# pchero/asterisk-tiresias

Hardware: AMD Instinct MI355X
Metric: fingerprints/sec + match latency p50, 8 kHz mono, 1/2/4/8 MI355X (higher is better)
Workload: dtype f32

## Files before the change

asterisk-tiresias_amd/csrc/tfp_kernels.hip:

```cpp
#include <hip/hip_runtime.h>
#include <hipcub/hipcub.hpp>
#include <type_traits>

#include "tfp_kernels.hpp"
#include "tfp_log.hpp"
#include "tfp_math.hpp"
#include "tfp_split.hpp"
#include "tfp_synth.hpp"

namespace tfp {


typedef float cf __attribute__((ext_vector_type(2)));

__device__ __forceinline__ cf swap(cf a) { return __builtin_shufflevector(a, a, 1, 0); }
__device__ __forceinline__ cf addsub(cf c, cf p) { return __builtin_elementwise_fma(p, cf{1.f, -1.f}, c); }
__device__ __forceinline__ cf subadd(cf c, cf p) { return __builtin_elementwise_fma(p, cf{-1.f, 1.f}, c); }

__device__ __forceinline__ cf cmul(cf a, cf w) {
  const cf p = a * cf{w.x, w.x};
  const cf q = swap(a) * cf{w.y, w.y};
  return subadd(p, q);
}

// ... 486 lines not shown
        micro[2 * g + cf] = micro_of_db(q);
        if (db) db[2 * g + cf] = q;
      }
    }
    wave_sync();
    if (__builtin_expect(dense_rows != 0, 0)) {
      const float lempty = aubio_log10_fast(0.f, S.logf);
      for (int i = lane; i < kWaveFrames * kFilters; i += 64) {
        const int r = i / kFilters, j = i % kFilters;
        if (((dense_rows >> r) & 1u) && T->mel_len[j] == 0) M.logs[r * kLogStride + j] = lempty;
      }
      dense_rows = 0;
      wave_sync();
    }
    c = cn;
    f0 = fn0;
  }
}

__device__ __forceinline__ void dft4_rot_a2(cf a0, cf a1, cf A2, cf a3, cf& X0, cf& X1, cf& X2, cf& X3) {
  const cf t0 = addsub(a0, swap(A2)), t1 = subadd(a0, swap(A2)), t2 = a1 + a3, t3 = a1 - a3;
  X0 = t0 + t2;
  X2 = t0 - t2;
  X1 = addsub(t1, swap(t3));
  X3 = subadd(t1, swap(t3));
}
__device__ __forceinline__ cf cmul_w2(cf a, float c) {
  const cf p = a * cf{c, c};
  return addsub(p, swap(p));
}
__device__ __forceinline__ cf cmul_w6(cf a, float d) {
  const cf p = a * cf{d, d};
  return subadd(p, swap(p));
}
__device__ __forceinline__ void dft16q(const cf (&w16)[10], const cf (&in)[16], cf (&out)[16]) {
  cf A[4][4];
#pragma unroll
  for (int n2 = 0; n2 < 4; n2++) dft4(in[n2], in[4 + n2], in[8 + n2], in[12 + n2], A[n2][0], A[n2][1], A[n2][2], A[n2][3]);
#pragma unroll
  for (int n2 = 1; n2 < 4; n2++)
#pragma unroll
    for (int k1 = 1; k1 < 4; k1++) {
      const int e = n2 * k1;
      if (e == 2) A[n2][k1] = cmul_w2(A[n2][k1], w16[2].x);
      else if (e == 6) A[n2][k1] = cmul_w6(A[n2][k1], w16[6].x);
      else if (e != 4) A[n2][k1] = cmul(A[n2][k1], w16[e]);
    }
#pragma unroll
  for (int k1 = 0; k1 < 4; k1++) {
    if (k1 == 2) dft4_rot_a2(A[0][k1], A[1][k1], A[2][k1], A[3][k1], out[k1], out[k1 + 4], out[k1 + 8], out[k1 + 12]);
    else dft4(A[0][k1], A[1][k1], A[2][k1], A[3][k1], out[k1], out[k1 + 4], out[k1 + 8], out[k1 + 12]);
  }
}

template <int LEN>
__device__ __forceinline__ float mel_sum_w(const float* __restrict__ N, const float4 (&wv)[LEN / 4], int st) {
  float4 nv[LEN / 4];
#pragma unroll
  for (int i = 0; i < LEN / 4; i++) nv[i] = *reinterpret_cast<const float4*>(N + st + 4 * i);
  float acc = 0.f;
#pragma unroll
  for (int i = 0; i < LEN / 4; i++) {
    const cf p01 = cf{nv[i].x, nv[i].y} * cf{wv[i].x, wv[i].y};
    const cf p23 = cf{nv[i].z, nv[i].w} * cf{wv[i].z, wv[i].w};
    acc = i == 0 ? p01.x : acc + p01.x;
    acc = acc + p01.y; acc = acc + p23.x; acc = acc + p23.y;
  }
  return acc;
}
template <int LEN>
__device__ __forceinline__ void load_w(const float* __restrict__ w, float4 (&wv)[LEN / 4]) {
#pragma unroll
  for (int i = 0; i < LEN / 4; i++) wv[i] = *reinterpret_cast<const float4*>(w + 64 * i);
}

#ifdef TFP_STAMPS
#define TFP_STAMP(i) const uint64_t ts##i = __builtin_amdgcn_s_memtime()
#define TFP_ACC(i, a, b) st[i] += ts##b - ts##a
#else
#define TFP_STAMP(i)
#define TFP_ACC(i, a, b)
#endif

template <int kPasses>
__global__ __launch_bounds__(64 * fp8_block_waves<kPasses>(), TFP_FP_WAVES) void fingerprint8k_kernel(
    const DspTables* __restrict__ T, const int16_t* __restrict__ pcm, const int64_t* __restrict__ sbeg,
    const int64_t* __restrict__ send, const int64_t* __restrict__ foff, const int32_t* __restrict__ toff,
    const int32_t* __restrict__ tclip, int32_t ntiles, int32_t* __restrict__ micro, double* __restrict__ db,
    float rare_thr, LogFix fx, int64_t single_ns) {
  constexpr int LA = 36, LB = 16, LC = 8;
  constexpr bool kSplitTail = kPasses >= 2;
#ifdef TFP_STAMPS
  const uint64_t t_entry = __builtin_amdgcn_s_memtime();
#endif
  const uint32_t rare_m1 = __builtin_bit_cast(uint32_t, rare_thr) - 1u;
  constexpr bool kPairFb = kPasses >= 2;
  constexpr int kBW = fp8_block_waves<kPasses>();
  using WaveT = WaveLds8;
  __shared__ __attribute__((aligned(16))) LdsTables S;
  __shared__ __attribute__((aligned(16))) WaveT WL[kBW];
  const int tid = threadIdx.x;
  const int wave = __builtin_amdgcn_readfirstlane(tid >> 6);
  const int lane = tid & 63, grp = lane >> 4, L = lane & 15;
  struct Tile {
    int c;
    int64_t f0, s0, ns;
    __amdgpu_buffer_rsrc_t rs;
    bool odd;
  };
  auto clip_rsrc = [&](int64_t s0, int64_t ns) {
    const uintptr_t a = reinterpret_cast<uintptr_t>(pcm + s0);
    const int16_t* base = reinterpret_cast<const int16_t*>(a & ~(uintptr_t)3);
    const int64_t bytes = (2 * ns + (int64_t)(a & 3) + 3) & ~(int64_t)3;
    return __builtin_amdgcn_make_buffer_rsrc(const_cast<int16_t*>(base), (short)0, (int)bytes, 0x00020000);
  };
  auto tile_of = [&](int b) {
    Tile t;
    if (single_ns >= 0) {
      t.c = 0;
      t.f0 = (int64_t)b * (4 * kPasses);
      t.s0 = 0;
      t.ns = single_ns;
    } else {
      t.c = __builtin_amdgcn_readfirstlane(tclip[b]);
      t.f0 = (int64_t)(b - toff[t.c]) * (4 * kPasses);
      t.s0 = sbeg[t.c];
      t.ns = send[t.c] - t.s0;
    }
    if constexpr (kPairFb) {
      t.rs = clip_rsrc(t.s0, t.ns);
      t.odd = (reinterpret_cast<uintptr_t>(pcm + t.s0) & 3) != 0;
    }
    return t;
  };
  auto fetch = [&](const Tile& t, int sub, bool valid, int4 (&pf)[kChunkRounds]) {
    const int16_t* clip = pcm + t.s0;
    const int64_t sb = (t.f0 + 4 * sub - 1) * kHop;
    const bool interior = valid && ((reinterpret_cast<uintptr_t>(clip) & 15) == 0) && sb >= 0 && sb + kPassSamples <= t.ns;
    if (interior) {
      const int4* src = reinterpret_cast<const int4*>(clip + sb);
#pragma unroll
      for (int r = 0; r < kChunkRounds; r++) {
        const int chunk = lane + 64 * r;
        pf[r] = (64 * r + 63 < kPassChunks || chunk < kPassChunks) ? src[chunk] : make_int4(0, 0, 0, 0);
      }
    } else if constexpr (kPasses == 1) {
      const bool aligned = (reinterpret_cast<uintptr_t>(clip) & 15) == 0;
#pragma unroll
      for (int r = 0; r < kChunkRounds; r++) {
        const int chunk = lane + 64 * r;
        const int64_t s0 = sb + 8 * chunk;
        int4 v = make_int4(0, 0, 0, 0);
        if (valid && chunk < kPassChunks && s0 + 8 > 0 && s0 < t.ns) {
          if (aligned && s0 >= 0 && s0 + 8 <= t.ns) v = *reinterpret_cast<const int4*>(clip + s0);
          else v = fetch_chunk_inline(clip, t.ns, s0);
        }
        pf[r] = v;
      }
    } else {
#pragma unroll
      for (int r = 0; r < kChunkRounds; r++) {
        const int chunk = lane + 64 * r;
        pf[r] = (valid && chunk < kPassChunks) ? fetch_chunk_checked(clip, t.ns, sb + 8 * chunk) : make_int4(0, 0, 0, 0);
      }
    }
  };

  auto fetchd = [&](const Tile& t, int sub, uint32_t (&pw)[16]) {
    if (t.odd) return;
    const __amdgpu_buffer_rsrc_t rs = t.rs;
    const int32_t fs = (int32_t)((t.f0 + 4 * sub - 1 + grp) * kHop) + 2 * L;
#pragma unroll
    for (int n1 = 0; n1 < 16; n1++) {
      const int32_t j = n1 < 8 ? 256 + 32 * n1 : 32 * (n1 - 8);
      pw[n1] = __builtin_amdgcn_raw_buffer_load_b32(rs, 2 * (fs + j), 0, 0);
    }
  };

  int4 pf[kChunkRounds];
  uint32_t pw[16];
  int b = blockIdx.x * kBW + wave;
  Tile cur = tile_of(b < ntiles ? b : 0);
  cf* winr = reinterpret_cast<cf*>(S.window);
  cf* twr = S.tw512;
  constexpr int kStage = 256;
  const int ts = tid < kStage ? tid : kStage - 1;
  const bool stager = tid < kStage;
  constexpr int kMsW = kPairFb ? kFbSteps * kFbPatterns : 16 * (LA + LB + LC);
  const float* const wsrc = kPairFb ? &T->fb_w[0][0][0] : T->ms_w;
  const int wL = (ts >> 1) & 15, wn1 = 2 * (ts >> 5) + (ts & 1);
  const int wj = (32 * wn1 + 2 * wL + 256) & 511;
  const float win0 = T->window_s[wj], win1 = T->window_s[wj + 1];
  const int tk2 = ts >> 5, tkk = (wL == 0 && tk2 == 0) ? 128 : wL + 16 * tk2;
  const float* tws = (ts & 1) ? T->tw512_im : T->tw512_re;
  const float twk = tws[tkk], twk2 = tws[256 - tkk];
  const int li = ts < 240 ? ts : 239, lk1 = 1 + li / 16, lL = li % 16;
  const float ltre = T->lane_tw_re[lk1][lL], ltim = T->lane_tw_im[lk1][lL];
  const int i10 = ts < 10 ? ts : 9;
  const float w16re = T->tw256_re[16 * i10], w16im = T->tw256_im[16 * i10];
  const int i80 = ts < kCoefs * kFilters ? ts : kCoefs * kFilters - 1;
  const float dctv = (&T->dct[0][0])[i80];
  const int i48 = ts < 48 ? ts : 47;
  const int msf = (&T->ms_filter[0][0])[i48], mss = (&T->ms_start[0][0])[i48];
  const int i3 = ts < 3 ? ts : 2;
  const int msl = T->ms_len[i3], mso = T->ms_woff[i3];
  const LogfEntry lge = logf_table()[ts & 15];
  float mw[(kMsW + kStage - 1) / kStage];
#pragma unroll
  for (int r = 0; r < (kMsW + kStage - 1) / kStage; r++) {
    int idx = ts + kStage * r;
    idx = idx < kMsW ? idx : kMsW - 1;
    if constexpr (kPairFb) {
      const int q = idx & 3, pat = (idx >> 2) & 15, s4 = idx >> 6;
      idx = ((2 * s4 + (q >> 1)) * kFbPatterns + pat) * 2 + (q & 1);
    }
    mw[r] = wsrc[idx];
  }
  const int mlen = T->mel_len[lane < kFilters ? lane : kFilters - 1];
  if constexpr (kPairFb) fetchd(cur, 0, pw);
  else fetch(cur, 0, b < ntiles, pf);
  if (stager) {
    winr[tid] = cf{win0, win1};
    twr[tid] = cf{twk, twk2};
  if (tid < 240) S.lane_tw[lk1 - 1][lL] = cf{ltre, ltim};
  if (tid < 10) S.w16[tid] = cf{w16re, w16im};
  if (tid < kCoefs * kFilters) (&S.dct[0][0])[tid] = dctv;
  if (tid < 48) {
    (&S.ms_filter[0][0])[tid] = msf;
    (&S.ms_start[0][0])[tid] = mss;
  }
  if (tid < 3) { S.ms_len[tid] = msl; S.ms_woff[tid] = mso; }
  if (tid < 16) S.logf[tid] = lge;
  if (kPairFb && tid < kLogf2Entries) S.logf2[tid] = logf2_entry(tid, logf_table());
  if (tid == 0) { S.c_defer = T->ms_c_defer; S.c_real[0] = T->ms_c_real[0]; S.c_real[1] = T->ms_c_real[1]; }
#pragma unroll
    for (int r = 0; r < (kMsW + kStage - 1) / kStage; r++) {
      const int idx = tid + kStage * r;
      if (idx < kMsW) S.ms_w[idx] = 0.5f * mw[r];
    }
  }
  const unsigned long long empty_filters = __ballot(lane < kFilters && mlen == 0);
  __syncthreads();
#ifdef TFP_STAMPS
  const uint64_t t_staged = __builtin_amdgcn_s_memtime();
#endif

  WaveT& M = WL[wave];
  cf* W = M.scratch[grp];
  float* N = reinterpret_cast<float*>(W) + 48 * (grp & 1);
  const int nwaves = gridDim.x * kBW;
  const int maxbin = T->ms_maxbin;
  const int fA = S.ms_filter[0][L], fB = S.ms_filter[1][L], fC = S.ms_filter[2][L];
  const bool c_real = fC >= 0 && (fC == S.c_real[0] || fC == S.c_real[1]);
  cf w16r[10];
#pragma unroll
  for (int e = 0; e < 10; e++)
    w16r[e] = cf{T->tw256_re[16 * e], T->tw256_im[16 * e]};
  cf ltw[15];
#pragma unroll
  for (int k1 = 1; k1 < 16; k1++) ltw[k1 - 1] = S.lane_tw[k1 - 1][L];
  const float lempty = aubio_log10_fast(0.f, S.logf);
  if constexpr (!kPairFb) {
    for (int i = lane; i < 4 * kPasses * kFilters; i += 64) {
      const int j = i % kFilters;
      if ((empty_filters >> j) & 1) M.logs[(i / kFilters) * kLogStride + j] = lempty;
    }
  }
  const float* fbb[kFbSegs];
  float* fbc[kFbSegs];
  float fbk[kFbSegs];
  cf dctl, dct9;
  const float* const fbrow = (grp < 2 ? M.xeven : reinterpret_cast<const float*>(M.scratch)) + (grp & 1) * kFbRow;
  float* const fblog = M.logs + 4 * grp * kFbNf;
  if constexpr (kPairFb) {
    const int lf = lane < kFbNf ? lane : lane - kFbNf, l9 = kFbNf - 4 + (lane & 3);
    dctl = cf{S.dct[0][lf], S.dct[1][lf]};
    dct9 = cf{S.dct[0][l9], S.dct[1][l9]};
#pragma unroll
    for (int k = 0; k < kFbSegs; k++) {
      fbb[k] = fbrow + 2 * (T->fb_bin[L][k] - kFbSegStart[k]);
      fbc[k] = fblog + T->fb_filter[L][k];
      fbk[k] = T->fb_new[L][k] ? 0.f : 1.f;
    }
  }

#ifdef TFP_STAMPS
  uint64_t st[7] = {0, 0, 0, 0, 0, 0, 0};
  uint64_t tprev = __builtin_amdgcn_s_memtime();
  const uint64_t tstart = tprev;
  int npass = 0;
#endif
  for (; b < ntiles; b += nwaves) {
    const int64_t nf = (cur.ns + kHop - 1) / kHop;
    const int bn = b + nwaves;
    const Tile nxt = bn < ntiles ? tile_of(bn) : cur;

    for (int sub = 0; sub < kPasses; sub++) {
      const int row = sub * 4 + grp;
      int oz = 0;
      asm volatile("" : "+v"(oz));
      wave_sync();
      TFP_STAMP(0);
      cf wreg[16];
#pragma unroll
      for (int i = 0; i < 8; i++) {
        const float4 w4 = *reinterpret_cast<const float4*>(winr + (i * 16 + L) * 2 + oz);
        wreg[2 * i] = cf{w4.x, w4.y};
        wreg[2 * i + 1] = cf{w4.z, w4.w};
      }
      if constexpr (!kPairFb) {
#pragma unroll
        for (int r = 0; r < kChunkRounds; r++) {
          const int chunk = lane + 64 * r;
          if (chunk < kPassChunks) *reinterpret_cast<int4*>(M.pcm + (chunk >> 5) * kHopStride + (chunk & 31) * 8) = pf[r];
        }
        if (sub < kPasses - 1) fetch(cur, sub + 1, true, pf);
        else fetch(nxt, 0, bn < ntiles, pf);
      }
      wave_sync();
      TFP_STAMP(1);
      const int16_t* hop0 = M.pcm + grp * kHopStride;
      cf z[16], Y[16];
      if constexpr (kPairFb) {
        const int64_t pb = (cur.f0 + 4 * sub - 1) * kHop;
        const int32_t fs = (int32_t)(pb + grp * kHop) + 2 * L;
        if (cur.odd) {
          const __amdgpu_buffer_rsrc_t rs = cur.rs;
#pragma unroll
          for (int n1 = 0; n1 < 16; n1++) {
            const int32_t j = n1 < 8 ? 256 + 32 * n1 : 32 * (n1 - 8);
            const uint32_t lo = __builtin_amdgcn_raw_buffer_load_b32(rs, 2 * (fs + j), 0, 0);
            const uint32_t hi = __builtin_amdgcn_raw_buffer_load_b32(rs, 2 * (fs + j) + 4, 0, 0);
            pw[n1] = (lo >> 16) | (hi << 16);
          }
        }
        if (pb < 0 || pb + kPassSamples > cur.ns) {
#pragma unroll
          for (int n1 = 0; n1 < 16; n1++) {
            const int32_t s0 = fs + (n1 < 8 ? 256 + 32 * n1 : 32 * (n1 - 8));
            const uint32_t lo = (s0 >= 0 && s0 < cur.ns) ? 0xffffu : 0u;
            const uint32_t hi = (s0 + 1 >= 0 && s0 + 1 < cur.ns) ? 0xffff0000u : 0u;
            pw[n1] &= lo | hi;
          }
        }
      }
#pragma unroll
      for (int n1 = 0; n1 < 16; n1++) {
        int32_t v;
        if constexpr (kPairFb) {
          v = (int32_t)pw[n1];
        } else {
          const int j = (32 * n1 + 2 * L + 256) & 511;
          const int hsel = n1 < 8 ? 1 : 0;
          v = *reinterpret_cast<const int32_t*>(hop0 + hsel * kHopStride + (j & 255));
        }
        z[n1] = cf{(float)(int16_t)(v & 0xffff), (float)(int16_t)(v >> 16)} * wreg[n1];
      }
      if constexpr (kPairFb) {
        if (sub < kPasses - 1) fetchd(cur, sub + 1, pw);
        else fetchd(nxt, 0, pw);
      }
      dft16q(w16r, z, Y);
#pragma unroll
      for (int k1 = 1; k1 < 16; k1++) Y[k1] = cmul(Y[k1], ltw[k1 - 1]);
      wave_sync();
      TFP_STAMP(2);
// ... 115 lines not shown
              if (st == 0) acc = p0;
              else if (st == kFbSegStart[k]) acc = __builtin_elementwise_fma(acc, cf{jk[k], jk[k]}, p0);
              else acc = acc + p0;
              acc = acc + p1;
            }
            seg[k] = acc;
          };
          using I0 = std::integral_constant<int, 0>;
          using I1 = std::integral_constant<int, 1>;
          using I2 = std::integral_constant<int, 2>;
          using I3 = std::integral_constant<int, 3>;
          static_assert(kFbSegs == 4, "four segments");
          load_seg(I0{});
          load_seg(I1{});
          asm volatile("" ::: "memory");
          sum_seg(I0{});
          load_seg(I2{});
          asm volatile("" ::: "memory");
          sum_seg(I1{});
          load_seg(I3{});
          asm volatile("" ::: "memory");
          sum_seg(I2{});
          sum_seg(I3{});
#pragma unroll
          for (int k = 0; k < kFbSegs; k++) {
            jc[k][doff] = seg[k].x;
            jc[k][doff + 2 * kFbNf] = seg[k].y;
          }
        };
        if (sub == 1) pair_fb(std::integral_constant<int, 0>{});
        else pair_fb(std::integral_constant<int, 1>{});
      }
#ifdef TFP_STAMPS
      const uint64_t ts5 = __builtin_amdgcn_s_memtime();
      st[0] += ts0 - tprev;
      TFP_ACC(1, 0, 1);
      TFP_ACC(2, 1, 2);
      TFP_ACC(3, 2, 3);
      TFP_ACC(4, 3, 4);
      TFP_ACC(5, 4, 5);
      tprev = ts5;
      npass++;
#endif
    }
    wave_sync();
    if constexpr (kPairFb) {
      constexpr int kFull = 8;
      static_assert(kWaveFrames * kFbNf == kFull * 2 * kFbNf && 2 * kFbNf - 64 == 4, "log rounds");
      cf* const prod = reinterpret_cast<cf*>(M.scratch);
      LogArg g[kFull];
      LogfEntry en[kFull];
#pragma unroll
      for (int r = 0; r < kFull; r++) g[r] = log_reduce(M.logs[2 * kFbNf * r + lane]);
#pragma unroll
      for (int r = 0; r < kFull; r++) en[r] = S.logf2[g[r].idx];
#pragma unroll
      for (int r = 0; r < kFull; r++) {
        const float l = log_finish(g[r], en[r]);
        prod[2 * kFbNf * r + lane] = cf{l, l} * dctl;
      }
      if (lane < kWaveFrames * 2) {
        const int i = 2 * kFbNf * (lane >> 2) + 64 + (lane & 3);
        const float l = aubio_log10_frexp(M.logs[i], S.logf2);
        prod[i] = cf{l, l} * dct9;
      }
    } else if (lane < 2 * 4 * kPasses) {
      const int f = S.c_real[lane & 1];
      if (f >= 0) {
        float* p = M.logs + (lane >> 1) * kLogStride + f;
        *p = aubio_log10_fast(*p, S.logf);
      }
    }
    wave_sync();
    if (lane < 2 * 4 * kPasses) {
      const int row = lane >> 1, cfi = lane & 1;
      const int64_t f = cur.f0 + row;
      if (f < nf) {
        float acc = 0.f;
        if constexpr (kPairFb) {
          const float* prow = reinterpret_cast<const float*>(M.scratch) + 2 * (2 * (row & 7) + (row >> 3)) * kFbNf + cfi;
#pragma unroll
          for (int i = 0; i < kFbNf; i++) acc = acc + prow[2 * i];
#pragma unroll
          for (int i = kFbNf; i < kFilters; i++) acc = acc + lempty * S.dct[cfi][i];
        } else {
          const float* lrow = M.logs + row * kLogStride;
#pragma unroll 8
          for (int i = 0; i < kFilters; i++) acc = acc + lrow[i] * S.dct[cfi][i];
        }
        const int64_t g = (single_ns >= 0 ? 0 : foff[cur.c]) + f;
        if constexpr (kSplitTail) {
          micro[2 * g + cfi] = __builtin_bit_cast(int32_t, acc);
        } else {
          const double q = db ? db_of_coef(acc, fx) : db_of_coef(acc);
          micro[2 * g + cfi] = micro_of_db(q);
          if (db) db[2 * g + cfi] = q;
        }
      }
    }
    wave_sync();
    cur = nxt;
  }
#ifdef TFP_STAMPS
  const uint64_t t_end = __builtin_amdgcn_s_memtime();
  if (lane == 0 && (blockIdx.x & 63) == 0)
    printf("stamps<%d> block %d wave %d passes %d | entry->staged %lu staged->loop %lu loop %lu after-last-pass %lu | "
           "lead %lu stage %lu fft1 %lu fft2 %lu split %lu mel %lu\n",
           kPasses, (int)blockIdx.x, wave, npass, (unsigned long)(t_staged - t_entry), (unsigned long)(tstart - t_staged),
           (unsigned long)(tprev - tstart), (unsigned long)(t_end - tprev), (unsigned long)st[0], (unsigned long)st[1],
           (unsigned long)st[2], (unsigned long)st[3], (unsigned long)st[4], (unsigned long)st[5]);
#endif
}

__global__ void finish_db_kernel(int32_t* __restrict__ micro, double* __restrict__ db, int64_t nvals, LogFix fx) {
  for (int64_t i = (int64_t)blockIdx.x * blockDim.x + threadIdx.x; i < nvals; i += (int64_t)gridDim.x * blockDim.x) {
    const float c = __builtin_bit_cast(float, micro[i]);
    const double q = db ? db_of_coef(c, fx) : db_of_coef(c);
    micro[i] = micro_of_db(q);
    if (db) db[i] = q;
  }
}

bool DspTables_fixed8k(const DspTables& t) {
  return t.ms_len[0] == 36 && t.ms_len[1] == 16 && t.ms_len[2] == 8 && t.ms_total == 16 * (36 + 16 + 8) &&
         t.ms_total <= kMsLds && t.ms_c_defer == 1 && t.ms_maxbin <= 2 * kFrameStride8 - 48 &&
         t.ms_filter[0][15] >= 0 && t.ms_filter[1][15] >= 0 && t.fb_ok == 1 && t.fb_nfilters == kFbNf &&
         t.tw256_im[32] == -t.tw256_re[32] && t.tw256_im[96] == t.tw256_re[96];
}

static int resident_blocks(const void* k, int waves = kBlockWaves) {
  int per = 0;
  (void)hipOccupancyMaxActiveBlocksPerMultiprocessor(&per, k, 64 * waves, 0);
  hipFuncAttributes a;
  if (hipFuncGetAttributes(&a, k) == hipSuccess) {
    const int vg = ((a.numRegs > 0 ? a.numRegs : 1) + 7) / 8 * 8;
    int by_vgpr = 512 / vg;
    if (by_vgpr > 8) by_vgpr = 8;
    by_vgpr = by_vgpr * 4 / waves;
    const int by_lds = a.sharedSizeBytes ? (int)((160 * 1024) / a.sharedSizeBytes) : 8;
    const int own = by_vgpr < by_lds ? by_vgpr : by_lds;
    if (per <= 0 || own < per) per = own;
  }
  return per > 0 ? per : 1;
}

hipError_t fp_launch_config(int device, FpLaunchCfg* cfg) {
  int cus = 0;
  hipError_t e = hipDeviceGetAttribute(&cus, hipDeviceAttributeMultiprocessorCount, device);
  if (e != hipSuccess) return e;
  auto cap = [&](const void* k, int waves = kBlockWaves) { return cus * resident_blocks(k, waves); };
  cfg->grid_cap_8k = cap(reinterpret_cast<const void*>(fingerprint8k_kernel<kTile8k / 4>), kBW8);
  cfg->grid_cap_8k_small = cap(reinterpret_cast<const void*>(fingerprint8k_kernel<1>));
  cfg->grid_cap_generic = cap(reinterpret_cast<const void*>(fingerprint_kernel<int16_t>));
  cfg->grid_cap_f32 = cap(reinterpret_cast<const void*>(fingerprint_kernel<float>));
  if (knob("TFP_DEBUG_OCC")) {
    int per = 0;
    (void)hipOccupancyMaxActiveBlocksPerMultiprocessor(&per, reinterpret_cast<const void*>(fingerprint8k_kernel<kTile8k / 4>),
                                                       64 * kBW8, 0);
    fprintf(stderr, "[tfp] fingerprint8k_kernel<%d>: %d blocks/CU (occupancy query %d), grid cap %d\n", kTile8k / 4,
            cfg->grid_cap_8k / cus, per, cfg->grid_cap_8k);
    hipFuncAttributes fa;
    if (hipFuncGetAttributes(&fa, reinterpret_cast<const void*>(fingerprint8k_kernel<kTile8k / 4>)) == hipSuccess)
      fprintf(stderr, "[tfp]   %d threads/block (max %d), %d VGPRs, %zu B LDS, %zu B scratch\n", 64 * kBW8,
              fa.maxThreadsPerBlock, fa.numRegs, fa.sharedSizeBytes, fa.localSizeBytes);
    int smem = 0, smem_optin = 0;
    (void)hipDeviceGetAttribute(&smem, hipDeviceAttributeMaxSharedMemoryPerBlock, device);
    (void)hipDeviceGetAttribute(&smem_optin, hipDeviceAttributeSharedMemPerBlockOptin, device);
    fprintf(stderr, "[tfp]   device: %d B LDS per block (opt-in %d)\n", smem, smem_optin);
  }
  if (const char* b = knob("TFP_FP_BLOCKS_PER_CU")) {
    const int n = atoi(b);
    if (n > 0 && cus * n < cfg->grid_cap_8k) cfg->grid_cap_8k = cus * n;
  }
  const char* g = knob("TFP_GENERIC");
  cfg->force_generic = g && atoi(g);
  const char* rt = knob("TFP_RARE_THR_LOG2");
  int rl = rt ? atoi(rt) : -98;
  rl = rl < -98 ? -98 : (rl > 100 ? 100 : rl);
  cfg->rare_thr = ldexpf(1.f, rl);
  return hipSuccess;
}

hipError_t launch_fingerprint(const FpLaunchCfg& cfg, const DspTables* d_tables, bool fixed8k, int32_t tile_frames,
                              const int16_t* d_pcm, const int64_t* d_sbeg, const int64_t* d_send, const int64_t* d_foff,
                              const int32_t* d_toff, const int32_t* d_tclip, int32_t ntiles, int64_t nframes,
                              int32_t* d_micro, double* d_db, hipStream_t s, const LogFix& fx, FpLaunchStats* stats,
                              int64_t single_ns) {
  const bool v8 = fixed8k && (tile_frames == 4 || !cfg.force_generic);
  if (v8 ? !(tile_frames == 4 || tile_frames == kTile8k) : tile_frames != kFramesPerBlock) return hipErrorInvalidValue;
  if (ntiles <= 0) return hipSuccess;
  const int cap = v8 ? (tile_frames == 4 ? cfg.grid_cap_8k_small : cfg.grid_cap_8k) : cfg.grid_cap_generic;
  if (cap <= 0) return hipErrorInvalidValue;
  const int bw = (v8 && tile_frames != 4) ? kBW8 : kBlockWaves;
  const int want = (ntiles + bw - 1) / bw;
  const int grid = want < cap ? want : cap;
  if (v8) {
    if (tile_frames == 4) {
      hipLaunchKernelGGL(fingerprint8k_kernel<1>, dim3(grid), dim3(kBlockThreads), 0, s, d_tables, d_pcm, d_sbeg, d_send,
                         d_foff, d_toff, d_tclip, ntiles, d_micro, d_db, cfg.rare_thr, fx, single_ns);
      if (stats) stats->small8k++;
    } else {
      hipLaunchKernelGGL(fingerprint8k_kernel<kTile8k / 4>, dim3(grid), dim3(64 * kBW8), 0, s, d_tables, d_pcm, d_sbeg,
                         d_send, d_foff, d_toff, d_tclip, ntiles, d_micro, d_db, cfg.rare_thr, fx, single_ns);
      if (stats) stats->throughput8k++;
      if (const hipError_t le = hipGetLastError(); le != hipSuccess) return le;
      const int64_t nv = 2 * nframes;
      int64_t g = (nv + 255) / 256;
      if (g > 8192) g = 8192;
      if (nv > 0) hipLaunchKernelGGL(finish_db_kernel, dim3((unsigned)g), dim3(256), 0, s, d_micro, d_db, nv, fx);
    }
    return hipGetLastError();
  }
  hipLaunchKernelGGL(fingerprint_kernel<int16_t>, dim3(grid), dim3(kBlockThreads), 0, s, d_tables, d_pcm, d_sbeg, d_send,
                     d_foff, d_toff, d_tclip, ntiles, d_micro, d_db, fx);
  if (stats) stats->generic_i16++;
  return hipGetLastError();
}

hipError_t launch_fingerprint_f32(const FpLaunchCfg& cfg, const DspTables* d_tables, const float* d_x,
                                  const int64_t* d_sbeg, const int64_t* d_send, const int64_t* d_foff,
                                  const int32_t* d_toff, const int32_t* d_tclip, int32_t ntiles, int32_t* d_micro,
                                  double* d_db, hipStream_t s, const LogFix& fx, FpLaunchStats* stats) {
  if (ntiles <= 0) return hipSuccess;
  if (cfg.grid_cap_f32 <= 0) return hipErrorInvalidValue;
  const int want = (ntiles + kBlockWaves - 1) / kBlockWaves;
  const int grid = want < cfg.grid_cap_f32 ? want : cfg.grid_cap_f32;
  hipLaunchKernelGGL(fingerprint_kernel<float>, dim3(grid), dim3(kBlockThreads), 0, s, d_tables, d_x, d_sbeg, d_send,
                     d_foff, d_toff, d_tclip, ntiles, d_micro, d_db, fx);
  if (stats) stats->generic_f32++;
  return hipGetLastError();
}

__global__ void synth_kernel(const SynthSpecDev* __restrict__ specs, int64_t spc, int16_t* __restrict__ out) {
  const int c = blockIdx.y;
  const SynthSpecDev sp = specs[c];
  const SynthClip p = synth_clip(sp.seed, sp.clip);
  for (int64_t s = (int64_t)blockIdx.x * blockDim.x + threadIdx.x; s < spc; s += (int64_t)gridDim.x * blockDim.x)
    out[(int64_t)c * spc + s] = synth_sample(p, sp.offset + s);
}

hipError_t launch_synth(const SynthSpecDev* d_specs, int32_t nclips, int64_t spc, int16_t* d_out, hipStream_t s) {
  if (nclips <= 0 || spc <= 0) return hipSuccess;
  int64_t bx = (spc + 255) / 256;
  if (bx > 256) bx = 256;
  hipLaunchKernelGGL(synth_kernel, dim3((unsigned)bx, nclips), dim3(256), 0, s, d_specs, spc, d_out);
  return hipGetLastError();
}

__global__ void index_keys_kernel(const int32_t* __restrict__ m1, const int32_t* __restrict__ clip,
                                  const int32_t* __restrict__ rank, int64_t n, int32_t* keys, int32_t* vals) {
  for (int64_t i = (int64_t)blockIdx.x * blockDim.x + threadIdx.x; i < n; i += (int64_t)gridDim.x * blockDim.x) {
    const int32_t v = m1[i];
    const bool live = rank[clip[i]] >= 0 && v != kNullMicro;
    keys[i] = live ? v : INT32_MAX;
    vals[i] = (int32_t)i;
  }
}

hipError_t launch_index_keys(const int32_t* st_m1, const int32_t* st_clip, const int32_t* rank_of_clip, int64_t n,
                             int32_t* keys, int32_t* vals, hipStream_t s) {
  if (n <= 0) return hipSuccess;
  hipLaunchKernelGGL(index_keys_kernel, dim3(2048), dim3(256), 0, s, st_m1, st_clip, rank_of_clip, n, keys, vals);
  return hipGetLastError();
}

__global__ void index_gather_kernel(const int32_t* __restrict__ sv, const int32_t* __restrict__ m2,
                                    const int32_t* __restrict__ clip, const int32_t* __restrict__ rank, int64_t n,
                                    int32_t* m2s, int32_t* cols) {
  for (int64_t i = (int64_t)blockIdx.x * blockDim.x + threadIdx.x; i < n; i += (int64_t)gridDim.x * blockDim.x) {
    const int32_t j = sv[i];
    m2s[i] = m2[j];
    cols[i] = rank[clip[j]];
  }
}

hipError_t launch_index_gather(const int32_t* sorted_vals, const int32_t* st_m2, const int32_t* st_clip,
                               const int32_t* rank_of_clip, int64_t n, int32_t* m2s, int32_t* cols, hipStream_t s) {
  if (n <= 0) return hipSuccess;
  hipLaunchKernelGGL(index_gather_kernel, dim3(2048), dim3(256), 0, s, sorted_vals, st_m2, st_clip, rank_of_clip, n,
                     m2s, cols);
  return hipGetLastError();
}

__device__ __forceinline__ int64_t lower_bound_i32(const int32_t* a, int64_t n, int64_t v) {
  int64_t lo = 0, hi = n;
  while (lo < hi) {
// ... 811 lines not shown
```

asterisk-tiresias_amd/csrc/tfp_kernels.hpp:

```cpp
#pragma once
#include <hip/hip_runtime.h>
#include <stdint.h>
#include <stdlib.h>
#include <string.h>

#include "tfp_math.hpp"
#include "tfp_tables.hpp"

namespace tfp {

inline const char* knob(const char* name) {
  const char* on = getenv("TFP_TEST_KNOBS");
  return on && *on && strcmp(on, "0") != 0 ? getenv(name) : nullptr;
}
inline const char* op_env(const char* name) {
  const char* v = getenv(name);
  return v && *v ? v : nullptr;
}

constexpr int kFramesPerBlock = 16;
constexpr int kTile8k = 16;
constexpr int64_t kDirectMaxSamples = (int64_t(1) << 30) - (int64_t(1) << 16);
constexpr int32_t kKeyOffset = 512;
constexpr int32_t kKeyRange = 1024;

struct FrameBox {
  int64_t L1, U1, L2, U2;
  int32_t k;
  int32_t flags;
};

struct SearchConsts {
  int32_t coefs;
  int32_t has_low, has_high;
  int32_t pad;
  double tole, thr_low, thr_high;
};

#ifdef __HIPCC__
__device__ __forceinline__ bool frame_key(const double* __restrict__ q, int64_t i, const SearchConsts& sc, int32_t& k) {
  const double q1 = q[2 * i];
  const double v1 = __builtin_isfinite(q1) ? q1 : 0.0;
  k = (v1 > -2147483649.0 && v1 < 2147483648.0) ? (int32_t)v1 : INT32_MIN;
  const double freq = (double)k;
  if (sc.has_low && freq < sc.thr_low) return false;
  if (sc.has_high && freq > sc.thr_high) return false;
  return __builtin_isfinite(freq - sc.tole) && __builtin_isfinite(freq + sc.tole);
}

__device__ __forceinline__ FrameBox frame_box(double q1, double q2, const SearchConsts& sc) {
  const double v1 = __builtin_isfinite(q1) ? q1 : 0.0;
  const int32_t ki = (v1 > -2147483649.0 && v1 < 2147483648.0) ? (int32_t)v1 : INT32_MIN;
  const double freq = (double)ki;
  FrameBox bx;
  bx.k = ki;
  bx.flags = 1;
  bx.L2 = bx.U2 = 0;
  if (sc.has_low && freq < sc.thr_low) bx.flags = 0;
  if (sc.has_high && freq > sc.thr_high) bx.flags = 0;
  const double lo = freq - sc.tole, hi = freq + sc.tole;
  if (!__builtin_isfinite(lo) || !__builtin_isfinite(hi)) bx.flags = 0;
  bx.L1 = fmt6_bound(lo);
  bx.U1 = fmt6_bound(hi);
  if (sc.coefs == 2 && bx.flags) {
    const double f2 = __builtin_isfinite(q2) ? q2 : 0.0;
    bool skip = false;
    if (sc.has_low && f2 < sc.thr_low) skip = true;
    else if (sc.has_high && f2 > sc.thr_high) skip = true;
    if (!skip) {
      const double lo2 = f2 - sc.tole, hi2 = f2 + sc.tole;
      if (!__builtin_isfinite(lo2) || !__builtin_isfinite(hi2)) bx.flags = 0;
      else {
        bx.L2 = fmt6_bound(lo2);
        bx.U2 = fmt6_bound(hi2);
        bx.flags |= 2;
      }
    }
  }
  return bx;
}
#endif

struct SynthSpecDev {
  uint64_t seed;
  int64_t clip;
  int64_t offset;
};

struct FpLaunchCfg {
  int32_t grid_cap_8k = 0;
  int32_t grid_cap_8k_small = 0;
  int32_t grid_cap_generic = 0;
  int32_t grid_cap_f32 = 0;
  bool force_generic = false;
  float rare_thr = 0x1p-98f;
};
struct FpLaunchStats {
  int64_t small8k = 0;
  int64_t throughput8k = 0;
  int64_t generic_i16 = 0;
  int64_t generic_f32 = 0;
};
hipError_t fp_launch_config(int device, FpLaunchCfg* cfg);
inline int32_t fp_tile_frames(const FpLaunchCfg& cfg, bool fixed8k, bool f32, bool small) {
  if (!fixed8k || f32) return kFramesPerBlock;
  if (small) return 4;
  return cfg.force_generic ? kFramesPerBlock : kTile8k;
}
bool DspTables_fixed8k(const DspTables& t);
hipError_t launch_fingerprint(const FpLaunchCfg& cfg, const DspTables* d_tables, bool fixed8k, int32_t tile_frames,
                              const int16_t* d_pcm, const int64_t* d_sbeg, const int64_t* d_send, const int64_t* d_foff,
                              const int32_t* d_toff, const int32_t* d_tclip, int32_t ntiles, int64_t nframes,
                              int32_t* d_micro, double* d_db, hipStream_t s, const LogFix& fx, FpLaunchStats* stats,
                              int64_t single_ns = -1);
hipError_t launch_fingerprint_f32(const FpLaunchCfg& cfg, const DspTables* d_tables, const float* d_x,
                                  const int64_t* d_sbeg, const int64_t* d_send, const int64_t* d_foff,
                                  const int32_t* d_toff, const int32_t* d_tclip, int32_t ntiles, int32_t* d_micro,
                                  double* d_db, hipStream_t s, const LogFix& fx, FpLaunchStats* stats);

hipError_t launch_synth(const SynthSpecDev* d_specs, int32_t nclips, int64_t spc, int16_t* d_out, hipStream_t s);

hipError_t launch_index_keys(const int32_t* st_m1, const int32_t* st_clip, const int32_t* rank_of_clip,
                             int64_t n, int32_t* keys, int32_t* vals, hipStream_t s);
hipError_t launch_index_gather(const int32_t* sorted_vals, const int32_t* st_m2, const int32_t* st_clip,
                               const int32_t* rank_of_clip, int64_t n, int32_t* m2s, int32_t* cols, hipStream_t s);
hipError_t launch_count_below(const int32_t* sorted_keys, int64_t n, int32_t bound, int64_t* out, hipStream_t s);
hipError_t radix_sort_pairs(void* temp, size_t* temp_bytes, const int32_t* kin, int32_t* kout, const int32_t* vin,
                            int32_t* vout, int64_t n, hipStream_t s);

hipError_t launch_prep_boxes(const double* d_q, int64_t nframes, SearchConsts sc, FrameBox* boxes, uint32_t* zero_words,
                             int32_t nzero, hipStream_t s);
struct VoteMeta;
hipError_t launch_key_mask(const double* d_q, SearchConsts sc, int64_t nf, uint32_t* d_mask ,
                           int32_t* d_maxc , VoteMeta* d_meta, hipStream_t s);
hipError_t launch_key_ranges_all(const int32_t* m1s, int64_t R, double tole, int64_t* d_rng_all ,
                                 hipStream_t s);
struct VoteMeta {
  int32_t ku;
  int32_t kp;
  int32_t ok;
  int32_t cls;
};
constexpr int32_t kVoteKpMax = ((kKeyRange + 1 + 15) / 16) * 16;
hipError_t launch_build_A(const double* d_q, SearchConsts sc, const int64_t* d_qoff, int32_t nq, int32_t Qp,
                          const uint32_t* d_mask, const int32_t* d_maxc, VoteMeta* d_meta, int32_t class_ku_max,
                          _Float16* d_A, _Float16* d_Bt , int32_t Cp,
                          hipStream_t s);
hipError_t launch_build_B(const uint32_t* d_mask , const uint32_t* d_bits ,
                          int32_t C, const VoteMeta* d_meta, int32_t Cp, _Float16* d_Bt ,
                          hipStream_t s);
int32_t vote_chunks(int32_t Cp);
hipError_t launch_vote_gemm(const _Float16* d_A, _Float16* d_Bt, int32_t Qp, int32_t Cp, const VoteMeta* d_meta,
                            const int32_t* d_tiekey, unsigned long long* d_part, unsigned long long* d_best,
                            const uint32_t* d_mask , const uint32_t* d_bits ,
                            int32_t C, hipStream_t s);

constexpr int kSmallQ = 8;
struct SmallQueries {
  int32_t nq;
  int32_t pad;
  int64_t qoff[kSmallQ + 1];
};
struct SmallResult {
  int32_t ku;
  int32_t bad;
};
constexpr int kSmallVoteClips = 1024;
inline int32_t small_vote_blocks(int32_t C) { return (C + kSmallVoteClips - 1) / kSmallVoteClips; }
inline size_t small_result_bytes(int32_t C) {
  return sizeof(SmallResult) + sizeof(unsigned long long) * kSmallQ * (size_t)small_vote_blocks(C);
}
TFP_HD unsigned long long* small_result_parts(SmallResult* r) { return reinterpret_cast<unsigned long long*>(r + 1); }
TFP_HD int32_t key_bits_words(int32_t C) { return (C + 127) / 128 * 4; }
hipError_t launch_key_bits(const int64_t* d_rng_all, const int32_t* cols, int32_t C, int64_t rows_bound, int32_t win,
                           int64_t direct, uint32_t* d_bits, hipStream_t s);
hipError_t launch_search_small(const double* d_q, const SmallQueries& sq, SearchConsts sc, const uint32_t* d_bits,
                               int32_t C, const int32_t* d_tiekey, SmallResult* h_out, hipStream_t s);

// ... 123 lines not shown
```

asterisk-tiresias_amd/csrc/tfp_math.hpp:

```cpp
#pragma once
#include <stdint.h>

#if defined(__HIPCC__) || defined(__HIP__)
#define TFP_HD __host__ __device__ inline
#else
#define TFP_HD static inline
#endif

namespace tfp {

TFP_HD uint32_t f2u(float f) { return __builtin_bit_cast(uint32_t, f); }
TFP_HD float u2f(uint32_t u) { return __builtin_bit_cast(float, u); }
TFP_HD uint64_t d2u(double d) { return __builtin_bit_cast(uint64_t, d); }
TFP_HD double u2d(uint64_t u) { return __builtin_bit_cast(double, u); }

constexpr int32_t kNullMicro = INT32_MIN;

struct LogfEntry { double invc, logc; };
#if defined(__HIPCC__) || defined(__HIP__)
__host__ __device__
#endif
inline const LogfEntry* logf_table() {
  static constexpr LogfEntry T[16] = {
      {0x1.661ec79f8f3bep+0, -0x1.57bf7808caadep-2}, {0x1.571ed4aaf883dp+0, -0x1.2bef0a7c06ddbp-2},
// ... 119 lines not shown
  int32_t hashed = 0;
  const uint32_t* bits = nullptr;
};

TFP_HD double log_fixed(double x, int32_t i, const LogFix& fx) {
  if (fx.n > 0 && (d2u(x) & 0x1fffffffull) == 0) {
    const uint32_t k = ((uint32_t)i << 23) | (uint32_t)((d2u(x) >> 29) & 0x7fffffu);
    if (fx.hashed) {
      if (fx.bits && !((fx.bits[k >> 5] >> (k & 31)) & 1u)) return log_acc(x);
      for (uint32_t h = log_fix_slot(k);; h = (h + 1) & ((1u << kLogFixHashBits) - 1)) {
        const uint32_t s = fx.key[h];
        if (s == k) return fx.val[h];
        if (s == kLogFixEmpty) break;
      }
      return log_acc(x);
    }
    int32_t lo = 0, hi = fx.n;
    while (lo < hi) {
      const int32_t mid = (lo + hi) >> 1;
      if (fx.key[mid] < k) lo = mid + 1; else hi = mid;
    }
    if (lo < fx.n && fx.key[lo] == k) return fx.val[lo];
  }
  return log_acc(x);
}

TFP_HD double log10_glibc_wrapper(double x, const LogFix& fx = LogFix{nullptr, nullptr, 0}) {
  const double two54 = 1.80143985094819840000e+16;
  const double ivln10 = 4.34294481903251816668e-01;
  const double log10_2hi = 3.01029995663611771306e-01;
  const double log10_2lo = 3.69423907715893078616e-13;
  uint64_t bits = d2u(x);
  int32_t hx = (int32_t)(bits >> 32);
  const uint32_t lx = (uint32_t)bits;
  int32_t k = 0;
  if (hx < 0x00100000) {
    if (((hx & 0x7fffffff) | (int32_t)lx) == 0) return -u2d(0x7ff0000000000000ull);
    if (hx < 0) return u2d(0x7ff8000000000000ull);
    k -= 54;
    x *= two54;
    bits = d2u(x);
    hx = (int32_t)(bits >> 32);
  }
  if (hx >= 0x7ff00000) return x + x;
  k += (hx >> 20) - 1023;
  const int32_t i = (int32_t)(((uint32_t)k & 0x80000000u) >> 31);
  hx = (hx & 0x000fffff) | ((0x3ff - i) << 20);
  const double y = (double)(k + i);
  x = u2d(((uint64_t)(uint32_t)hx << 32) | (d2u(x) & 0xffffffffull));
  const double z = y * log10_2lo + ivln10 * log_fixed(x, i, fx);
  return z + y * log10_2hi;
}

TFP_HD double db_of_coef(float c, const LogFix& fx = LogFix{nullptr, nullptr, 0}) {
  const double a = (double)c;
  return 10.0 * log10_glibc_wrapper(a < 0.0 ? -a : a, fx);
}

TFP_HD int64_t fmt6(double x) {
  const double p = x * 1e6;
  const double e = __builtin_fma(x, 1e6, -p);
  double n = __builtin_rint(p);
  const double d = p - n;
  if (d == 0.5 || d == -0.5) {
    if (e > 0.0) n = p + 0.5;
    else if (e < 0.0) n = p - 0.5;
  }
  return (int64_t)n;
}

constexpr int64_t kBoundSat = (int64_t)1 << 60;
TFP_HD int64_t fmt6_bound(double x) {
  if (!(x < 1e12)) return kBoundSat;
  if (!(x > -1e12)) return -kBoundSat;
  return fmt6(x);
}

TFP_HD int32_t micro_of_db(double q) {
  const double inf = u2d(0x7ff0000000000000ull);
  if (!(q > -inf && q < inf)) return kNullMicro;
  return (int32_t)fmt6(q);
}

}
```

Before: 2.319 billion.

## Fuse fast table-based dB/micro finish into the 8k throughput fingerprint kernel

Adds a fused variant of the throughput 8k kernel, used when no dB output is requested. It computes the quantized log10 micro value in-kernel with a 128-entry LDS table and a short polynomial, instead of writing raw coefficients for a separate split-tail finishing pass. Values whose rounding falls too close to a half-integer go to a slow exact path, which keeps results bit-exact while removing the extra kernel and its memory round trip. It also precomputes the constant empty-filter DCT terms per lane. The cost is more LDS and registers, which may lower occupancy.

```diff
diff --git a/asterisk-tiresias_amd/csrc/tfp_kernels.hip b/asterisk-tiresias_amd/csrc/tfp_kernels.hip
--- a/asterisk-tiresias_amd/csrc/tfp_kernels.hip
+++ b/asterisk-tiresias_amd/csrc/tfp_kernels.hip
@@ -592,14 +592,17 @@
 #define TFP_ACC(i, a, b)
 #endif
 
-template <int kPasses>
+__device__ __noinline__ int32_t finish_slow(float c) { return micro_of_db(db_of_coef(c)); }
+
+template <int kPasses, bool kFused = false>
 __global__ __launch_bounds__(64 * fp8_block_waves<kPasses>(), TFP_FP_WAVES) void fingerprint8k_kernel(
     const DspTables* __restrict__ T, const int16_t* __restrict__ pcm, const int64_t* __restrict__ sbeg,
     const int64_t* __restrict__ send, const int64_t* __restrict__ foff, const int32_t* __restrict__ toff,
     const int32_t* __restrict__ tclip, int32_t ntiles, int32_t* __restrict__ micro, double* __restrict__ db,
-    float rare_thr, LogFix fx, int64_t single_ns) {
+    float rare_thr, LogFix fx, int64_t single_ns, double fin_thr) {
+  static_assert(!kFused || kPasses >= 2, "the fused finish belongs to the throughput tile");
   constexpr int LA = 36, LB = 16, LC = 8;
-  constexpr bool kSplitTail = kPasses >= 2;
+  constexpr bool kSplitTail = kPasses >= 2 && !kFused;
 #ifdef TFP_STAMPS
   const uint64_t t_entry = __builtin_amdgcn_s_memtime();
 #endif
@@ -609,6 +612,7 @@
   using WaveT = WaveLds8;
   __shared__ __attribute__((aligned(16))) LdsTables S;
   __shared__ __attribute__((aligned(16))) WaveT WL[kBW];
+  __shared__ __attribute__((aligned(16))) FinEntry FT[kFused ? 128 : 1];
   const int tid = threadIdx.x;
   const int wave = __builtin_amdgcn_readfirstlane(tid >> 6);
   const int lane = tid & 63, grp = lane >> 4, L = lane & 15;
@@ -715,6 +719,8 @@
   const int i3 = ts < 3 ? ts : 2;
   const int msl = T->ms_len[i3], mso = T->ms_woff[i3];
   const LogfEntry lge = logf_table()[ts & 15];
+  FinEntry fte;
+  if constexpr (kFused) fte = fin_table()[ts & 127];
   float mw[(kMsW + kStage - 1) / kStage];
 #pragma unroll
   for (int r = 0; r < (kMsW + kStage - 1) / kStage; r++) {
@@ -742,6 +748,9 @@
   if (tid < 3) { S.ms_len[tid] = msl; S.ms_woff[tid] = mso; }
   if (tid < 16) S.logf[tid] = lge;
   if (kPairFb && tid < kLogf2Entries) S.logf2[tid] = logf2_entry(tid, logf_table());
+  if constexpr (kFused) {
+    if (tid < 128) FT[tid] = fte;
+  }
   if (tid == 0) { S.c_defer = T->ms_c_defer; S.c_real[0] = T->ms_c_real[0]; S.c_real[1] = T->ms_c_real[1]; }
 #pragma unroll
     for (int r = 0; r < (kMsW + kStage - 1) / kStage; r++) {
@@ -792,6 +801,11 @@
       fbc[k] = fblog + T->fb_filter[L][k];
       fbk[k] = T->fb_new[L][k] ? 0.f : 1.f;
     }
+  }
+  float lemp[kFilters - kFbNf];
+  if constexpr (kFused) {
+#pragma unroll
+    for (int i = kFbNf; i < kFilters; i++) lemp[i - kFbNf] = lempty * S.dct[lane & 1][i];
   }
 
 #ifdef TFP_STAMPS
@@ -1073,14 +1087,24 @@
 #pragma unroll
           for (int i = 0; i < kFbNf; i++) acc = acc + prow[2 * i];
 #pragma unroll
-          for (int i = kFbNf; i < kFilters; i++) acc = acc + lempty * S.dct[cfi][i];
+          for (int i = kFbNf; i < kFilters; i++) {
+            if constexpr (kFused) acc = acc + lemp[i - kFbNf];
+            else acc = acc + lempty * S.dct[cfi][i];
+          }
         } else {
           const float* lrow = M.logs + row * kLogStride;
 #pragma unroll 8
           for (int i = 0; i < kFilters; i++) acc = acc + lrow[i] * S.dct[cfi][i];
         }
         const int64_t g = (single_ns >= 0 ? 0 : foff[cur.c]) + f;
-        if constexpr (kSplitTail) {
+        if constexpr (kFused) {
+          bool und;
+          int32_t mv = micro_of_coef_fast(acc, &und, FT, fin_thr);
+          if (__builtin_expect(__any(und), 0)) {
+            if (und) mv = finish_slow(acc);
+          }
+          micro[2 * g + cfi] = mv;
+        } else if constexpr (kSplitTail) {
           micro[2 * g + cfi] = __builtin_bit_cast(int32_t, acc);
         } else {
           const double q = db ? db_of_coef(acc, fx) : db_of_coef(acc);
@@ -1140,7 +1164,8 @@
   hipError_t e = hipDeviceGetAttribute(&cus, hipDeviceAttributeMultiprocessorCount, device);
   if (e != hipSuccess) return e;
   auto cap = [&](const void* k, int waves = kBlockWaves) { return cus * resident_blocks(k, waves); };
-  cfg->grid_cap_8k = cap(reinterpret_cast<const void*>(fingerprint8k_kernel<kTile8k / 4>), kBW8);
+  cfg->grid_cap_8k = cap(reinterpret_cast<const void*>(fingerprint8k_kernel<kTile8k / 4, true>), kBW8);
+  cfg->grid_cap_8k_db = cap(reinterpret_cast<const void*>(fingerprint8k_kernel<kTile8k / 4>), kBW8);
   cfg->grid_cap_8k_small = cap(reinterpret_cast<const void*>(fingerprint8k_kernel<1>));
   cfg->grid_cap_generic = cap(reinterpret_cast<const void*>(fingerprint_kernel<int16_t>));
   cfg->grid_cap_f32 = cap(reinterpret_cast<const void*>(fingerprint_kernel<float>));
@@ -1162,6 +1187,7 @@
   if (const char* b = knob("TFP_FP_BLOCKS_PER_CU")) {
     const int n = atoi(b);
     if (n > 0 && cus * n < cfg->grid_cap_8k) cfg->grid_cap_8k = cus * n;
+    if (n > 0 && cus * n < cfg->grid_cap_8k_db) cfg->grid_cap_8k_db = cus * n;
   }
   const char* g = knob("TFP_GENERIC");
   cfg->force_generic = g && atoi(g);
@@ -1169,6 +1195,10 @@
   int rl = rt ? atoi(rt) : -98;
   rl = rl < -98 ? -98 : (rl > 100 ? 100 : rl);
   cfg->rare_thr = ldexpf(1.f, rl);
+  const char* fm = knob("TFP_FINISH_MARGIN_LOG2");
+  int ml = fm ? atoi(fm) : -22;
+  ml = ml < -22 ? -22 : (ml > 0 ? 0 : ml);
+  cfg->fin_thr = 0.5 - ldexp(1.0, ml);
   return hipSuccess;
 }
 
@@ -1180,7 +1210,9 @@
   const bool v8 = fixed8k && (tile_frames == 4 || !cfg.force_generic);
   if (v8 ? !(tile_frames == 4 || tile_frames == kTile8k) : tile_frames != kFramesPerBlock) return hipErrorInvalidValue;
   if (ntiles <= 0) return hipSuccess;
-  const int cap = v8 ? (tile_frames == 4 ? cfg.grid_cap_8k_small : cfg.grid_cap_8k) : cfg.grid_cap_generic;
+  const bool fused = d_db == nullptr;
+  const int cap = v8 ? (tile_frames == 4 ? cfg.grid_cap_8k_small : fused ? cfg.grid_cap_8k : cfg.grid_cap_8k_db)
+                     : cfg.grid_cap_generic;
   if (cap <= 0) return hipErrorInvalidValue;
   const int bw = (v8 && tile_frames != 4) ? kBW8 : kBlockWaves;
   const int want = (ntiles + bw - 1) / bw;
@@ -1188,11 +1220,16 @@
   if (v8) {
     if (tile_frames == 4) {
       hipLaunchKernelGGL(fingerprint8k_kernel<1>, dim3(grid), dim3(kBlockThreads), 0, s, d_tables, d_pcm, d_sbeg, d_send,
-                         d_foff, d_toff, d_tclip, ntiles, d_micro, d_db, cfg.rare_thr, fx, single_ns);
+                         d_foff, d_toff, d_tclip, ntiles, d_micro, d_db, cfg.rare_thr, fx, single_ns, cfg.fin_thr);
       if (stats) stats->small8k++;
+    } else if (fused) {
+      hipLaunchKernelGGL((fingerprint8k_kernel<kTile8k / 4, true>), dim3(grid), dim3(64 * kBW8), 0, s, d_tables, d_pcm,
+                         d_sbeg, d_send, d_foff, d_toff, d_tclip, ntiles, d_micro, d_db, cfg.rare_thr, fx, single_ns,
+                         cfg.fin_thr);
+      if (stats) stats->throughput8k++;
     } else {
       hipLaunchKernelGGL(fingerprint8k_kernel<kTile8k / 4>, dim3(grid), dim3(64 * kBW8), 0, s, d_tables, d_pcm, d_sbeg,
-                         d_send, d_foff, d_toff, d_tclip, ntiles, d_micro, d_db, cfg.rare_thr, fx, single_ns);
+                         d_send, d_foff, d_toff, d_tclip, ntiles, d_micro, d_db, cfg.rare_thr, fx, single_ns, cfg.fin_thr);
       if (stats) stats->throughput8k++;
       if (const hipError_t le = hipGetLastError(); le != hipSuccess) return le;
       const int64_t nv = 2 * nframes;
diff --git a/asterisk-tiresias_amd/csrc/tfp_kernels.hpp b/asterisk-tiresias_amd/csrc/tfp_kernels.hpp
--- a/asterisk-tiresias_amd/csrc/tfp_kernels.hpp
+++ b/asterisk-tiresias_amd/csrc/tfp_kernels.hpp
@@ -89,11 +89,13 @@
 
 struct FpLaunchCfg {
   int32_t grid_cap_8k = 0;
+  int32_t grid_cap_8k_db = 0;
   int32_t grid_cap_8k_small = 0;
   int32_t grid_cap_generic = 0;
   int32_t grid_cap_f32 = 0;
   bool force_generic = false;
   float rare_thr = 0x1p-98f;
+  double fin_thr = kFinThr;
 };
 struct FpLaunchStats {
   int64_t small8k = 0;
diff --git a/asterisk-tiresias_amd/csrc/tfp_math.hpp b/asterisk-tiresias_amd/csrc/tfp_math.hpp
--- a/asterisk-tiresias_amd/csrc/tfp_math.hpp
+++ b/asterisk-tiresias_amd/csrc/tfp_math.hpp
@@ -225,4 +225,107 @@
   return (int32_t)fmt6(q);
 }
 
-}
+struct FinEntry { double invc, l10c; };
+constexpr double kFinMargin = 0x1p-22;
+constexpr double kFinThr = 0.5 - kFinMargin;
+#if defined(__HIPCC__) || defined(__HIP__)
+__host__ __device__
+#endif
+inline const FinEntry* fin_table() {
+  static constexpr FinEntry T[128] = {
+      {0x1.fe01fe0000000p-1, 0x1.156832e30da53p-6}, {0x1.fa11ca0000000p-1, 0x1.9e7fd7c55e623p-5},
+      {0x1.f6310a0000000p-1, 0x1.58162d40b97dep-4}, {0x1.f25f640000000p-1, 0x1.dfe0ed39f1e47p-4},
+      {0x1.ee9c800000000p-1, 0x1.335224efb067cp-3}, {0x1.eae8080000000p-1, 0x1.7632307771537p-3},
+      {0x1.e741aa0000000p-1, 0x1.b892826586226p-3}, {0x1.e3a9180000000p-1, 0x1.fa74dbdcccda9p-3},
+      {0x1.e01e020000000p-1, 0x1.1deda15a5edcbp-2}, {0x1.dca01e0000000p-1, 0x1.3e63b6ed6b043p-2},
+      {0x1.d92f220000000p-1, 0x1.5e9d992a97c67p-2}, {0x1.d5cac80000000p-1, 0x1.7e9c1be8e9f4bp-2},
+      {0x1.d272ca0000000p-1, 0x1.9e60213ea9aedp-2}, {0x1.cf26e60000000p-1, 0x1.bdea733b7a662p-2},
+      {0x1.cbe6da0000000p-1, 0x1.dd3be95c238fcp-2}, {0x1.c8b2660000000p-1, 0x1.fc555531014b4p-2},
+      {0x1.c5894e0000000p-1, 0x1.0d9bb71970a54p-1}, {0x1.c26b540000000p-1, 0x1.1cf185e18bf34p-1},
+      {0x1.bf583e0000000p-1, 0x1.2c2c75282d466p-1}, {0x1.bc4fd60000000p-1, 0x1.3b4cd50ba1060p-1},
+      {0x1.b951e20000000p-1, 0x1.4a530f3fc3f47p-1}, {0x1.b65e2e0000000p-1, 0x1.593f750f5f56fp-1},
+      {0x1.b374840000000p-1, 0x1.6812673e01d0ep-1}, {0x1.b094b40000000p-1, 0x1.76cc2d4bc0c3fp-1},
+      {0x1.adbe880000000p-1, 0x1.856d32939d748p-1}, {0x1.aaf1d20000000p-1, 0x1.93f5be7187247p-1},
+      {0x1.a82e660000000p-1, 0x1.a2661265c70aep-1}, {0x1.a574100000000p-1, 0x1.b0be9e8b61fdep-1},
+      {0x1.a2c2a80000000p-1, 0x1.beff98cb092f1p-1}, {0x1.a01a020000000p-1, 0x1.cd29505c669b8p-1},
+      {0x1.9d79f20000000p-1, 0x1.db3c18faabaf5p-1}, {0x1.9ae24e0000000p-1, 0x1.e938401b283bcp-1},
+      {0x1.9852f00000000p-1, 0x1.f71e01bb5b478p-1}, {0x1.95cbb00000000p-1, 0x1.0276d44e55ee6p+0},
+      {0x1.934c680000000p-1, 0x1.0953bc4afda64p+0}, {0x1.90d4f20000000p-1, 0x1.1025dcaeacebfp+0},
+      {0x1.8e65280000000p-1, 0x1.16ed5b4806afbp+0}, {0x1.8bfce80000000p-1, 0x1.1daa54a22568ep+0},
+      {0x1.899c100000000p-1, 0x1.245ce6fdec20bp+0}, {0x1.87427c0000000p-1, 0x1.2b05380492b06p+0},
+      {0x1.84f00c0000000p-1, 0x1.31a363cfe97f2p+0}, {0x1.82a4a00000000p-1, 0x1.38378817745afp+0},
+      {0x1.8060180000000p-1, 0x1.3ec1c433c3033p+0}, {0x1.7e22560000000p-1, 0x1.454233500f5a0p+0},
+      {0x1.7beb3a0000000p-1, 0x1.4bb8f7f69887bp+0}, {0x1.79baa60000000p-1, 0x1.522630791ff9fp+0},
+      {0x1.7790820000000p-1, 0x1.5889eaf114c56p+0}, {0x1.756cac0000000p-1, 0x1.5ee454632ab89p+0},
+      {0x1.734f0c0000000p-1, 0x1.65357db8b662fp+0}, {0x1.7137860000000p-1, 0x1.6b7d851179863p+0},
+      {0x1.6f26020000000p-1, 0x1.71bc7de36c150p+0}, {0x1.6d1a620000000p-1, 0x1.77f28f1a0a259p+0},
+      {0x1.6b14900000000p-1, 0x1.7e1fc8bc801a2p+0}, {0x1.6914740000000p-1, 0x1.8444420cd482dp+0},
+      {0x1.6719f40000000p-1, 0x1.8a6019b5b4b00p+0}, {0x1.6524f80000000p-1, 0x1.9073698477f5ap+0},
+      {0x1.63356c0000000p-1, 0x1.967e3ffd63d1dp+0}, {0x1.614b360000000p-1, 0x1.9c80bf7f282a9p+0},
+      {0x1.5f66440000000p-1, 0x1.a27af27bdaceep+0}, {0x1.5d867c0000000p-1, 0x1.a86cfdb226461p+0},
+      {0x1.5babcc0000000p-1, 0x1.ae56edb2b2247p+0}, {0x1.59d6200000000p-1, 0x1.b438d65a41ed1p+0},
+      {0x1.5805600000000p-1, 0x1.ba12d975b48a8p+0}, {0x1.56397c0000000p-1, 0x1.bfe5001ea5306p+0},
+      {0x1.54725e0000000p-1, 0x1.c5af67c7bef85p+0}, {0x1.52aff60000000p-1, 0x1.cb721b5c78451p+0},
+      {0x1.50f22e0000000p-1, 0x1.d12d3a58ef232p+0}, {0x1.4f38f60000000p-1, 0x1.d6e0d18152b87p+0},
+      {0x1.4d843c0000000p-1, 0x1.dc8cf50c5686ap+0}, {0x1.4bd3ee0000000p-1, 0x1.e231ba1cc050bp+0},
+      {0x1.4a27fa0000000p-1, 0x1.e7cf36c2f45f2p+0}, {0x1.4880520000000p-1, 0x1.ed657474cc47bp+0},
+      {0x1.46dce40000000p-1, 0x1.f2f48aee491c9p+0}, {0x1.453d9e0000000p-1, 0x1.f87c92dd74abdp+0},
+      {0x1.43a2740000000p-1, 0x1.fdfd91471a2dfp+0}, {0x1.420b520000000p-1, 0x1.01bbd3ad73423p+1},
+      {0x1.40782e0000000p-1, 0x1.04756a5809cc9p+1}, {0x1.3ee8f40000000p-1, 0x1.072b9e1387f5cp+1},
+      {0x1.3d5d9a0000000p-1, 0x1.09de6f59c6068p+1}, {0x1.3bd60e0000000p-1, 0x1.0c8decf0bbc8dp+1},
+      {0x1.3a52440000000p-1, 0x1.0f3a1b7f6fc4ep+1}, {0x1.38d22e0000000p-1, 0x1.11e30384cc624p+1},
+      {0x1.3755be0000000p-1, 0x1.1488addbb9786p+1}, {0x1.35dce60000000p-1, 0x1.172b23bbac056p+1},
+      {0x1.34679a0000000p-1, 0x1.19ca6b1e5250ep+1}, {0x1.32f5ce0000000p-1, 0x1.1c668a499df32p+1},
+      {0x1.3187760000000p-1, 0x1.1eff87d049ae6p+1}, {0x1.301c820000000p-1, 0x1.219571e22b4dfp+1},
+      {0x1.2eb4ea0000000p-1, 0x1.2428486ea5062p+1}, {0x1.2d50a00000000p-1, 0x1.26b816a268838p+1},
+      {0x1.2bef980000000p-1, 0x1.2944e45559daep+1}, {0x1.2a91ca0000000p-1, 0x1.2bceb23c08e97p+1},
+      {0x1.2937260000000p-1, 0x1.2e55902e6f18ap+1}, {0x1.27dfa40000000p-1, 0x1.30d97f6f8a42dp+1},
+      {0x1.268b380000000p-1, 0x1.335a88fcc4d58p+1}, {0x1.2539d80000000p-1, 0x1.35d8b259deaf6p+1},
+      {0x1.23eb7a0000000p-1, 0x1.3854014a9e27ep+1}, {0x1.22a0120000000p-1, 0x1.3acc7fa68d7e9p+1},
+      {0x1.2157980000000p-1, 0x1.3d422fe80f84cp+1}, {0x1.2012020000000p-1, 0x1.3fb51895645e8p+1},
+      {0x1.1ecf440000000p-1, 0x1.42254456c1ac6p+1}, {0x1.1d8f560000000p-1, 0x1.4492b65e4a89dp+1},
+      {0x1.1c52300000000p-1, 0x1.46fd720f17927p+1}, {0x1.1b17c60000000p-1, 0x1.496582d85a773p+1},
+      {0x1.19e0120000000p-1, 0x1.4bcae8a87894cp+1}, {0x1.18ab080000000p-1, 0x1.4e2daf70b4657p+1},
+      {0x1.1778a20000000p-1, 0x1.508dd78821b1ep+1}, {0x1.1648d60000000p-1, 0x1.52eb6964a5658p+1},
+      {0x1.151b9a0000000p-1, 0x1.55466dc07eab5p+1}, {0x1.13f0e80000000p-1, 0x1.579ee58bb0d35p+1},
+      {0x1.12c8b80000000p-1, 0x1.59f4d5e44424dp+1}, {0x1.11a3020000000p-1, 0x1.5c48441c26e13p+1},
+      {0x1.107fbc0000000p-1, 0x1.5e9939cdf2b90p+1}, {0x1.0f5ee00000000p-1, 0x1.60e7b8a87698ep+1},
+      {0x1.0e40660000000p-1, 0x1.6333c69b0ebccp+1}, {0x1.0d24460000000p-1, 0x1.657d69ca2055dp+1},
+      {0x1.0c0a780000000p-1, 0x1.67c4a88f5e97cp+1}, {0x1.0af2f80000000p-1, 0x1.6a098125ab909p+1},
+      {0x1.09ddba0000000p-1, 0x1.6c4c0295239bap+1}, {0x1.08cabc0000000p-1, 0x1.6e8c2740515a0p+1},
+      {0x1.07b9f20000000p-1, 0x1.70c9fea01234ep+1}, {0x1.06ab5a0000000p-1, 0x1.7305835cc1db7p+1},
+      {0x1.059eea0000000p-1, 0x1.753ec1210fc73p+1}, {0x1.04949c0000000p-1, 0x1.7775bb5796076p+1},
+      {0x1.038c6c0000000p-1, 0x1.79aa71483df15p+1}, {0x1.0286500000000p-1, 0x1.7bdcef3681af8p+1},
+      {0x1.0182440000000p-1, 0x1.7e0d34bb1c4c5p+1}, {0x1.0080400000000p-1, 0x1.803b4a2f38bd8p+1},
+  };
+  return T;
+}
+
+TFP_HD int32_t micro_of_coef_fast(float c, bool* undecided, const FinEntry* T = fin_table(), double thr = kFinThr) {
+  const double K_HI = 0x1.8151824c75800p+1, K_LO = 0x1.fabf59b5d80b8p-45;
+  const double A1 = 0x1.15f2ced384f29p+2, A2 = -0x1.15f2ced384f29p+1, A3 = 0x1.729913c4b1436p+0;
+  const double A4 = -0x1.15f2ced384f29p+0, A5 = 0x1.bcb7b1526e50ep-1, A6 = -0x1.729913c4b1436p-1;
+  const uint32_t ix = f2u(c) & 0x7fffffffu;
+  const uint32_t be = ix >> 23;
+  const bool null = ix == 0 || be == 255;
+  const uint32_t mant = ix & 0x7fffffu;
+  const FinEntry t = T[mant >> 16];
+  const double m = u2d(0x3ff0000000000000ull | ((uint64_t)mant << 29));
+  const double e = (double)((int32_t)be - 127);
+  const double r = __builtin_fma(m, t.invc, -1.0);
+  double P = __builtin_fma(A6, r, A5);
+  P = __builtin_fma(P, r, A4);
+  P = __builtin_fma(P, r, A3);
+  P = __builtin_fma(P, r, A2);
+  P = __builtin_fma(P, r, A1);
+  P = P * r;
+  const double t1 = __builtin_fma(e, K_LO, t.l10c);
+  const double q = __builtin_fma(e, K_HI, t1 + P);
+  const double p = q * 1e6;
+  const double n = __builtin_rint(p);
+  const double d = p - n;
+  *undecided = !null && !(be != 0 && (d < 0.0 ? -d : d) < thr);
+  return null ? kNullMicro : (int32_t)n;
+}
+
+}
```

After: 2.375 billion (median of 6 runs). +2.4%, better.
